# BUBLET/uav-airvision

Measured on AMD Instinct MI355X. Metric: stereo frames/sec (LK+stereo+MSCKF-update) at 752x480, higher is better.
Workload: dtype u8/int32 windows, f32 normal equations

## Files before the change

### uav_airvision_amd/csrc/av_common.h

```cpp
#pragma once
#include <hip/hip_runtime.h>
#include <stdint.h>
#include <stdio.h>
#include <string.h>

#include "../../include/airvision.h"

#define AV_EXPORT extern "C" __attribute__((visibility("default")))

#include "av_resources.h"
#define AV_LAUNCH_CHECK()                                                                         \
    do {                                                                                          \
        hipError_t e_ = hipGetLastError();                                                        \
        if (e_ != hipSuccess) {                                                                   \
            av_set_error("kernel launch failed: %s (%s:%d)", hipGetErrorString(e_), __FILE__, __LINE__); \
            return AV_E_HIP;                                                                      \
        }                                                                                         \
    } while (0)

struct PyrGeom {
    int levels;
    int w[AV_MAX_LEVELS], h[AV_MAX_LEVELS], pitch[AV_MAX_LEVELS];
    int off[AV_MAX_LEVELS];
};
PyrGeom av_make_geom(const av_pyr_layout& l);

struct CamModel {
    double fx, fy, cx, cy, k1, k2, p1, p2;
    int model;
};

#define AV_KP_RASTER_BITS 19
#define AV_KP_RASTER_BITS_WIDE 24
static_assert((1 << AV_KP_RASTER_BITS_WIDE) == AV_MAX_IMAGE_PIXELS, "the wide keypoint word holds every raster of the largest image");
static_assert(((254ull << AV_KP_RASTER_BITS_WIDE) | ((1ull << AV_KP_RASTER_BITS_WIDE) - 1ull)) < 0xFFFFFFFFull, "the largest keypoint word stays below the sentinel");
inline int av_kp_raster_bits(int w, int h) { return (int64_t)w * h <= (1 << AV_KP_RASTER_BITS) ? AV_KP_RASTER_BITS : AV_KP_RASTER_BITS_WIDE; }

#ifdef __HIPCC__
#define AV_HD __host__ __device__
#else
#define AV_HD
#endif
AV_HD inline uint32_t av_ransac_mix(uint32_t x)
{
    x ^= x >> 16; x *= 0x7feb352du; x ^= x >> 15; x *= 0x846ca68bu; x ^= x >> 16;
    return x;
}
AV_HD inline uint32_t av_ransac_hash_inl(uint32_t seed, uint32_t frame, uint32_t camera, uint32_t k, uint32_t draw)
{
    return av_ransac_mix(av_ransac_mix(av_ransac_mix(seed + 0x9e3779b9u) ^ frame) ^ (camera << 16 | k << 1 | draw));
}

#ifdef __HIPCC__
__device__ __forceinline__ void av_mask_box(uint8_t* m, int w, int h, float px, float py, int j, uint8_t val)
{
    int fx = (int)px, fy = (int)py;
    if (fx < 3 || fy < 3) return;
    int yy = fy - 3 + j / 7, xx = fx - 3 + j % 7;
    if (yy < h && xx < w) m[(size_t)yy * w + xx] = val;
}

__device__ __forceinline__ int av_reflect101(int p, int len)
{
    if (p < 0) p = -p;
    if (p >= len) p = 2 * len - 2 - p;
    return p;
}
__device__ __forceinline__ int av_reflect101_any(int p, int len)
{
    if ((unsigned)p < (unsigned)len) return p;
    if (len == 1) return 0;
    do { p = p < 0 ? -p : 2 * len - 2 - p; } while ((unsigned)p >= (unsigned)len);
    return p;
}

__device__ __forceinline__ void av_undistort_fisheye(const CamModel& c, const double* R, double u, double v, double& ox, double& oy)
{
    const double pwx = (u - c.cx) / c.fx, pwy = (v - c.cy) / c.fy;
    const double half_pi = 3.1415926535897932384626433832795 / 2.;
    double theta_d = sqrt(pwx * pwx + pwy * pwy);
    theta_d = fmin(fmax(-half_pi, theta_d), half_pi);
    bool converged = false;
    double theta = theta_d, scale = 0.0;
    if (fabs(theta_d) > 1e-8) {
#pragma unroll 1
        for (int j = 0; j < 10; ++j) {
            const double theta2 = theta * theta, theta4 = theta2 * theta2, theta6 = theta4 * theta2, theta8 = theta6 * theta2;
            const double k0_theta2 = c.k1 * theta2, k1_theta4 = c.k2 * theta4, k2_theta6 = c.p1 * theta6, k3_theta8 = c.p2 * theta8;
            const double theta_fix = (theta * (1 + k0_theta2 + k1_theta4 + k2_theta6 + k3_theta8) - theta_d) /
                                     (1 + 3 * k0_theta2 + 5 * k1_theta4 + 7 * k2_theta6 + 9 * k3_theta8);
            theta = theta - theta_fix;
            if (fabs(theta_fix) < 1e-8) { converged = true; break; }
        }
        scale = tan(theta) / theta_d;
// ... 103 lines not shown
    const int64_t e = av_frame_entry(p, f.g);
    if (e < 0) return false;
    f.src = (f.cam ? p.src1 : p.src0) + (p.src_listed ? e : (int64_t)f.g) * p.src_stride;
    f.dst = (f.cam ? p.dst1 : p.dst0) + e * p.dst_stride;
    return true;
}
#endif

inline bool av_frames_vec16(const FrameSet& src, const FrameSet& dst, int n_groups)
{
    auto al16 = [](const void* p) { return (reinterpret_cast<uintptr_t>(p) & 15) == 0; };
    const bool strides16 = (n_groups == 1 && !src.map && !dst.map) || ((src.stride & 15) == 0 && (dst.stride & 15) == 0);
    return strides16 && al16(src.base[0]) && al16(src.base[1]) && al16(dst.base[0]) && al16(dst.base[1]);
}
inline bool av_spans_overlap(const void* in, int64_t in_stride, int64_t in_bytes, const void* out, int64_t out_stride, int64_t out_bytes, int n)
{
    const uintptr_t i0 = reinterpret_cast<uintptr_t>(in), i1 = i0 + (uint64_t)(n - 1) * in_stride + in_bytes;
    const uintptr_t o0 = reinterpret_cast<uintptr_t>(out), o1 = o0 + (uint64_t)(n - 1) * out_stride + out_bytes;
    return o0 < i1 && i0 < o1;
}

int av_launch_pyramid(const FrameSet& img, int n_groups,
                      const PyrGeom& g, uint8_t* pyr_base, int64_t stream_stride, int64_t slot_stride, int slot0, int slot1,
                      hipStream_t st, bool write_level0 = true, bool* wrote_level0 = nullptr);

struct LKParams {
    int win, max_iter;
    double eps2, min_eig;
};
int av_launch_lk(const ImgView& I, const ImgView& J, int n_set, const PyrGeom& g,
                 const float* prev, float* next, uint8_t* status, const int* count, int cap, int launch_pts,
                 const LKParams& p, hipStream_t st, const int* index = nullptr);

void av_fast_tiles(int w, int h, int* tiles, int* tile_cap);
int av_launch_fast(const ImgView& src, const PyrGeom* g, const uint8_t* mask, int64_t mask_stride,
                   int n_img, int w, int h, int threshold, int raster_bits,
                   uint32_t* kp, int* count, int cap,
                   uint32_t* tile_kp, int* tile_count,
                   int* overflow, int stat_stride, hipStream_t st);

struct RansacStage {
    int S, NT, MAXF, w, h;
    CamModel cam[2];
    const float* prev_p0; const float* prev_p1;
    long long* cur_id; int* cur_life; float* cur_p0; float* cur_p1; int* cur_cell; const int* cur_src; int* cur_count;
    uint8_t* mask;
    const double* Rpc;
    const int* frame_no;
    const int* slot_cur;
    int* counts;
    double thr; int N; uint32_t seed;
};
int av_launch_ransac_stage(const RansacStage& a, hipStream_t st);

int av_clahe_check(int w, int h, double clip_limit, int tiles_x, int tiles_y, const char* who);
int av_launch_clahe(const FrameSet& src, const FrameSet& dst, int n_groups, int w, int h, double clip_limit, int tiles_x, int tiles_y,
                    uint8_t* lut, hipStream_t st);

int av_pixfmt_bytes(int fmt);
int av_pixfmt_packed_depth(int fmt);
bool av_pixfmt_packed_csi2(int fmt);
bool av_pixfmt_is_bayer(int fmt);
const char* av_pixfmt_name(int fmt);
int av_pixfmt_check(int fmt, int shift, const char* who);
int av_pixfmt_check_size(int fmt, int w, int h, const char* who);
int av_launch_to_gray8(const FrameSet& src, const FrameSet& dst, int n_groups, int w, int h, int fmt, int shift, hipStream_t st, const FrameSet* mosaic = nullptr);
int av_launch_unpack_to_gray8(const FrameSet& src, const FrameSet& dst, int n_groups, int w, int h, int fmt, int shift, hipStream_t st);
int av_launch_bayer_to_gray8(const FrameSet& src, const FrameSet& dst, int n_groups, int w, int h, int fmt, int shift, hipStream_t st);
int av_launch_downscale(const FrameSet& src, const FrameSet& dst, int n_groups, int W, int H, int f, hipStream_t st);
int av_launch_photometric(const FrameSet& src, const FrameSet& dst, int n_groups, int w, int h, const uint16_t* resp0, const uint16_t* resp1,
                          const uint16_t* gain0, const uint16_t* gain1, const uint16_t* k0, const uint16_t* k1, hipStream_t st);
struct Range16 {
    int mode, lo, hi, ppm_lo, ppm_hi, min_span;
    uint32_t* hist; uint32_t* rec; int32_t* range_out;
};
int av_range16_check(int mode, int lo, int hi, int ppm_lo, int ppm_hi, int min_span, const char* who);
int av_launch_gray16_range(const FrameSet& src, const FrameSet& dst, int n_groups, int w, int h, const Range16& r, hipStream_t st);
```

### uav_airvision_amd/csrc/fast.hip

```cpp
#include <stdlib.h>

#include "av_common.h"

namespace {

constexpr int TW = 64, TH = 48;
constexpr int PW = TW + 8, PH = TH + 8;
constexpr int PWD = PW / 4;
constexpr int SP = PW, SH = TH + 2;
constexpr int SPD = SP / 4;
constexpr int TCAP = TW * TH / 4;

struct FastArgs {
    const uint8_t* img;
    int64_t img_stride;
    int img_pitch;
    int border;
    const uint8_t* mask;
    int64_t mask_stride;
    int w, h, threshold;
    int rbits;
    uint32_t* kp; int* count; int cap;
    uint32_t* tile_kp; int* tile_count;
    int* overflow; int stat_stride;
    int n_img, tiles_x, tiles_y;
    const int* index;
};

typedef short av_s2 __attribute__((ext_vector_type(2)));
typedef _Float16 av_h2 __attribute__((ext_vector_type(2)));
typedef unsigned short av_us2 __attribute__((ext_vector_type(2)));
__device__ __forceinline__ av_h2 h2_swap(av_h2 x) { return __builtin_shufflevector(x, x, 1, 0); }
__device__ __forceinline__ av_h2 h2_min(av_h2 a, av_h2 b) { return __builtin_elementwise_minimum(a, b); }
__device__ __forceinline__ av_h2 h2_max(av_h2 a, av_h2 b) { return __builtin_elementwise_maximum(a, b); }
__device__ __forceinline__ av_h2 h2_min3(av_h2 a, av_h2 b, av_h2 c) { return __builtin_elementwise_minimum(__builtin_elementwise_minimum(a, b), c); }
__device__ __forceinline__ av_h2 h2_max3(av_h2 a, av_h2 b, av_h2 c) { return __builtin_elementwise_maximum(__builtin_elementwise_maximum(a, b), c); }
__device__ __forceinline__ int fast_score(const uint8_t* c, int t)
{
    constexpr int DX[16] = {0, 1, 2, 3, 3, 3, 2, 1, 0, -1, -2, -3, -3, -3, -2, -1};
// ... 324 lines not shown
```

### uav_airvision_amd/csrc/frontend.hip

```cpp
#include <math.h>

#include <deque>
#include <mutex>
#include <new>
#include <vector>

#include "av_common.h"

namespace {

constexpr int CNT_BEFORE = 0, CNT_TRACKED = 1, CNT_MATCHED = 2, CNT_FAST = 3, CNT_CAND = 4, CNT_NEW = 5, CNT_PUB = 6, CNT_OVF = 7;
constexpr int NCNT = 8;
constexpr unsigned long long LIFE_MAX = 0xFFFFFFull;

struct FeDev {
    int S, w, h, C, grid_row, grid_col, gh, gw, gmin, gmax;
    int MAXF;
    int NT;
    int CC;
    int cell_cap;
    int rbits;
    int NSORT;
    CamModel cam0, cam1;
    double R0to1[9], E[9], I3[9];
    double epi_thr;
    long long* feat_id[2]; int* feat_life[2]; float* feat_p0[2]; float* feat_p1[2]; int* feat_cell[2]; int* n_feat[2];
    long long* next_id; int* first_frame;
    const double* Hmat;
    float* trk_prev; float* trk_next; uint8_t* trk_status; int* trk_count;
    int* sv_src; float* sv_p0; float* sv_init; float* sv_p1; uint8_t* sv_st; float* sv_back; uint8_t* sv_st2; int* sv_count;
    long long* cur_id; int* cur_life; float* cur_p0; float* cur_p1; int* cur_cell; int* cur_count;
    int* cur_src;
    uint32_t* cell_kp; int* cell_count; uint8_t* mask;
    uint32_t* tile_kp; int* tile_count; int n_tiles, tile_cap;
    uint32_t* cand_key; float* cand_p0; float* cand_init; float* cand_p1; uint8_t* cand_st; float* cand_back; uint8_t* cand_st2;
    uint8_t* cand_inl; int* cand_off; int* cand_count;
    int* r1_list; int* r2_list; int* r1_count; int* r2_count;
    long long* out_ids; double* out_uv; int* out_n;
    int* counters;
    const int* slot_cur;
    const uint8_t* smask0; const uint8_t* smask1;
};

__device__ __forceinline__ bool fe_idle(const FeDev& d, int s) { return d.slot_cur != nullptr && d.slot_cur[s] < 0; }

__global__ __launch_bounds__(64) void restart_kernel(FeDev d, const int* list, int n, int* rs_counts)
{
    const int i = blockIdx.x * 64 + threadIdx.x;
    if (i >= n) return;
    const int s = list[i];
    if (s < 0 || s >= d.S) return;
    d.first_frame[s] = 1; d.next_id[s] = 0;
    d.n_feat[0][s] = 0; d.n_feat[1][s] = 0;
    for (int k = 0; k < NCNT; ++k) d.counters[s * NCNT + k] = 0;
    if (rs_counts) for (int k = 0; k < 4; ++k) rs_counts[4 * (size_t)s + k] = 0;
}

__device__ __forceinline__ bool smask_valid(const FeDev& d, const uint8_t* m, float x, float y)
{
    const int xi = min(max((int)x, 0), d.w - 1), yi = min(max((int)y, 0), d.h - 1);
    return m[(size_t)yi * d.w + xi] != 0;
}

__device__ __forceinline__ int cell_of(const FeDev& d, float x, float y)
{
    return (int)(y / (float)d.gh) * d.grid_col + (int)(x / (float)d.gw);
// ... 67 lines not shown
    d.trk_prev[2 * t] = x; d.trk_prev[2 * t + 1] = y;
    d.trk_next[2 * t] = (float)(h0 / h2); d.trk_next[2 * t + 1] = (float)(h1 / h2);
}

__global__ __launch_bounds__(256) void track_gate_kernel(FeDev d)
{
    __shared__ int lds4[4];
    const int s = blockIdx.x;
    if (fe_idle(d, s)) return;
    const int n = d.trk_count[s];
    int base = 0;
    for (int i0 = 0; i0 < n; i0 += NTB) {
        const int i = i0 + threadIdx.x;
        const size_t t = (size_t)s * d.NT + i;
        bool keep = false; float x = 0, y = 0;
        if (i < n) {
            x = d.trk_next[2 * t]; y = d.trk_next[2 * t + 1];
            keep = d.trk_status[t] != 0 && !(x < 0 || x > (float)(d.w - 1) || y < 0 || y > (float)(d.h - 1));
            if (keep && d.smask0) keep = smask_valid(d, d.smask0, x, y);
        }
        int pos = block_ordered_pos(keep, base, lds4);
        if (keep) {
            const size_t o = (size_t)s * d.NT + pos;
            d.sv_src[o] = i;
            d.sv_p0[2 * o] = x; d.sv_p0[2 * o + 1] = y;
            float ix, iy;
            stereo_init(d, x, y, ix, iy);
            d.sv_init[2 * o] = ix; d.sv_init[2 * o + 1] = iy;
            d.sv_p1[2 * o] = ix; d.sv_p1[2 * o + 1] = iy;
            d.sv_back[2 * o] = x; d.sv_back[2 * o + 1] = y;
        }
    }
    if (threadIdx.x == 0) { d.sv_count[s] = base; d.counters[s * NCNT + CNT_TRACKED] = base; }
}

__device__ __forceinline__ void mask_box(const FeDev& d, uint8_t* m, float px, float py, int j, uint8_t val)
{
    av_mask_box(m, d.w, d.h, px, py, j, val);
}

__global__ __launch_bounds__(256) void rebin_kernel(FeDev d, int par)
{
    __shared__ int lds4[4];
    const int s = blockIdx.x;
    if (fe_idle(d, s)) return;
    const int n = d.sv_count[s];
    int base = 0;
    for (int i0 = 0; i0 < n; i0 += NTB) {
        const int i = i0 + threadIdx.x;
        const size_t t = (size_t)s * d.NT + i;
        bool keep = false;
        if (i < n)
            keep = stereo_gate(d, d.sv_p0[2 * t], d.sv_p0[2 * t + 1], d.sv_init[2 * t], d.sv_init[2 * t + 1],
                               d.sv_p1[2 * t], d.sv_p1[2 * t + 1], d.sv_st[t], d.sv_back[2 * t], d.sv_back[2 * t + 1]);
        int pos = block_ordered_pos(keep, base, lds4);
        if (keep) {
            const size_t o = (size_t)s * d.NT + pos;
            const size_t src = (size_t)s * d.MAXF + d.sv_src[t];
            d.cur_id[o] = d.feat_id[par][src];
            d.cur_life[o] = d.feat_life[par][src] + 1;
            float x = d.sv_p0[2 * t], y = d.sv_p0[2 * t + 1];
            d.cur_p0[2 * o] = x; d.cur_p0[2 * o + 1] = y;
            d.cur_p1[2 * o] = d.sv_p1[2 * t]; d.cur_p1[2 * o + 1] = d.sv_p1[2 * t + 1];
            d.cur_cell[o] = cell_of(d, x, y);
            if (d.cur_src) d.cur_src[o] = d.sv_src[t];
        }
    }
    if (threadIdx.x == 0) { d.cur_count[s] = base; d.counters[s * NCNT + CNT_MATCHED] = base; }
    if (d.cur_src) return;
    __syncthreads();
    uint8_t* m = d.mask + (size_t)s * d.w * d.h;
    for (int q = threadIdx.x; q < base * 49; q += NTB) {
        int f = q / 49, j = q - f * 49;
        const size_t o = (size_t)s * d.NT + f;
        mask_box(d, m, d.cur_p0[2 * o], d.cur_p0[2 * o + 1], j, 0);
    }
}

__device__ __forceinline__ unsigned long long wave_max_u64(unsigned long long v)
{
#pragma unroll
    for (int m = 32; m >= 1; m >>= 1) {
        unsigned long long o = __shfl_xor(v, m, 64);
        v = o > v ? o : v;
    }
    return v;
}

__global__ __launch_bounds__(256) void select_kernel(FeDev d)
{
    extern __shared__ int sm[];
    int* cnt = sm;
    int* off = sm + d.C;
    int* ccnt = off + d.C + 1;
    int* tpre = ccnt + d.C;
    const int s = blockIdx.x;
    if (fe_idle(d, s)) return;
    const int ts = d.slot_cur ? d.slot_cur[s] : s;
    const bool first = d.first_frame[s] != 0;
    {
        __shared__ int tmax;
        const int nt = d.n_tiles;
        const uint32_t rmask = (1u << d.rbits) - 1u;
        constexpr int BK = 32, BU = 5;
        if (threadIdx.x == 0) tmax = 0;
        for (int c = threadIdx.x; c < d.C; c += NTB) ccnt[c] = 0;
        __syncthreads();
        int mx = 0;
        for (int t = threadIdx.x; t < nt; t += NTB) { const int n = d.tile_count[(size_t)ts * nt + t]; tpre[t] = n; mx = max(mx, n); }
        if (mx > 0) atomicMax(&tmax, mx);
        __syncthreads();
        const int maxcount = tmax;
        for (int kb = 0; kb < maxcount; kb += BK)
            for (int j0 = threadIdx.x; j0 < nt * BK; j0 += NTB * BU) {
                uint32_t word[BU]; int x[BU], y[BU]; bool ok[BU]; uint8_t mk[BU];
#pragma unroll
                for (int u = 0; u < BU; ++u) {
                    const int j = j0 + NTB * u, t = j / BK, k = kb + (j % BK);
                    ok[u] = j < nt * BK && k < tpre[min(t, nt - 1)];
                    word[u] = ok[u] ? d.tile_kp[((size_t)ts * nt + t) * d.tile_cap + k] : 0u;
                }
#pragma unroll
                for (int u = 0; u < BU; ++u) {
                    const uint32_t raster = rmask - (word[u] & rmask);
                    y[u] = (int)(raster / (uint32_t)d.w); x[u] = (int)(raster % (uint32_t)d.w);
                    mk[u] = ok[u] ? d.mask[(size_t)s * d.w * d.h + (size_t)y[u] * d.w + x[u]] : (uint8_t)0;
                }
#pragma unroll
                for (int u = 0; u < BU; ++u) {
                    if (!ok[u] || mk[u] == 0) continue;
                    const int cell = (y[u] / d.gh) * d.grid_col + x[u] / d.gw;
                    const int idx = atomicAdd(&ccnt[cell], 1);
                    if (idx < d.cell_cap) d.cell_kp[((size_t)s * d.C + cell) * d.cell_cap + idx] = word[u];
                    else atomicOr(&d.counters[s * NCNT + CNT_OVF], 2);
                }
            }
        __threadfence_block();
        __syncthreads();
        if (threadIdx.x == 0) { int tot = 0; for (int c = 0; c < d.C; ++c) tot += ccnt[c]; d.counters[s * NCNT + CNT_FAST] = tot; }
    }
    for (int c = threadIdx.x; c < d.C; c += NTB) {
        int n = min(ccnt[c], d.cell_cap);
        cnt[c] = first ? n : min(n, d.gmax);
    }
    __syncthreads();
    if (threadIdx.x == 0) {
        int acc = 0;
        for (int c = 0; c < d.C; ++c) {
            off[c] = acc;
            int take = cnt[c];
            if (acc + take > d.CC) { take = d.CC - acc; atomicOr(&d.counters[s * NCNT + CNT_OVF], 4); }
            cnt[c] = take;
            acc += take;
        }
        off[d.C] = acc;
        d.cand_count[s] = acc;
        d.counters[s * NCNT + CNT_CAND] = acc;
    }
    __syncthreads();
    for (int c = threadIdx.x; c <= d.C; c += NTB) d.cand_off[s * (d.C + 1) + c] = off[c];
    {
        __shared__ int r1n;
        if (threadIdx.x == 0) r1n = 0;
// ... 189 lines not shown
        const unsigned long long k = keys[j];
        const int c = (int)(k >> 48), ins = (int)(k & 0xFFFFFFull);
        const int rank = j - cell_start[c];
        if (rank >= d.gmax) continue;
        const size_t o = (size_t)s * d.MAXF + out_start[c] + rank;
        if (ins < T) {
            const size_t t = (size_t)s * d.NT + ins;
            d.feat_id[nxt][o] = d.cur_id[t];
            d.feat_life[nxt][o] = d.cur_life[t];
            d.feat_p0[nxt][2 * o] = d.cur_p0[2 * t]; d.feat_p0[nxt][2 * o + 1] = d.cur_p0[2 * t + 1];
            d.feat_p1[nxt][2 * o] = d.cur_p1[2 * t]; d.feat_p1[nxt][2 * o + 1] = d.cur_p1[2 * t + 1];
        } else {
            const size_t q = (size_t)s * d.CC + new_cand[ins - T];
            d.feat_id[nxt][o] = id0 + (ins - T);
            d.feat_life[nxt][o] = 1;
            d.feat_p0[nxt][2 * o] = d.cand_p0[2 * q]; d.feat_p0[nxt][2 * o + 1] = d.cand_p0[2 * q + 1];
            d.feat_p1[nxt][2 * o] = d.cand_p1[2 * q]; d.feat_p1[nxt][2 * o + 1] = d.cand_p1[2 * q + 1];
            flags[0] = 1;
        }
        d.feat_cell[nxt][o] = c;
    }
    __syncthreads();
    const int n_out = out_start[d.C];
    const bool f64 = flags[0] != 0;
    for (int j = threadIdx.x; j < n_out; j += NTB) {
        const size_t o = (size_t)s * d.MAXF + j;
        double u0, v0, u1, v1;
        av_undistort(d.cam0, d.I3, (double)d.feat_p0[nxt][2 * o], (double)d.feat_p0[nxt][2 * o + 1], u0, v0);
        av_undistort(d.cam1, d.I3, (double)d.feat_p1[nxt][2 * o], (double)d.feat_p1[nxt][2 * o + 1], u1, v1);
        if (!f64) { u0 = (double)(float)u0; v0 = (double)(float)v0; }
        d.out_ids[o] = d.feat_id[nxt][o];
        d.out_uv[4 * o] = u0; d.out_uv[4 * o + 1] = v0;
        d.out_uv[4 * o + 2] = (double)(float)u1; d.out_uv[4 * o + 3] = (double)(float)v1;
    }
    uint8_t* m = d.mask + (size_t)s * d.w * d.h;
    for (int q = threadIdx.x; q < T * 49; q += NTB) {
        int f = q / 49, j = q - f * 49;
        const size_t o = (size_t)s * d.NT + f;
        mask_box(d, m, d.cur_p0[2 * o], d.cur_p0[2 * o + 1], j, 1);
    }
    if (threadIdx.x == 0) {
        d.n_feat[nxt][s] = n_out;
        d.out_n[s] = n_out;
        d.next_id[s] = id0 + n_new;
        d.first_frame[s] = 0;
        d.counters[s * NCNT + CNT_NEW] = n_new;
        d.counters[s * NCNT + CNT_PUB] = n_out;
    }
}

struct ImuSample { double t; double w[3]; };

struct StreamHost {
    std::deque<ImuSample> imu;
    std::mutex mu;
    double t_prev = 0.0;
    bool first = true;
    int frame = 0;
};

inline void mat3_mul(const double* A, const double* B, double* o)
{
    for (int i = 0; i < 3; ++i)
        for (int j = 0; j < 3; ++j) o[i * 3 + j] = (A[i * 3 + 0] * B[0 * 3 + j] + A[i * 3 + 1] * B[1 * 3 + j]) + A[i * 3 + 2] * B[2 * 3 + j];
}

inline void rodrigues(const double* r, double* R)
{
    double theta = sqrt((r[0] * r[0] + r[1] * r[1]) + r[2] * r[2]);
    if (theta < 2.220446049250313e-16) { for (int i = 0; i < 9; ++i) R[i] = (i % 4 == 0) ? 1.0 : 0.0; return; }
    double c = cos(theta), s = sin(theta), c1 = 1. - c, it = 1. / theta;
    double x = r[0] * it, y = r[1] * it, z = r[2] * it;
// ... 260 lines not shown
    }
    fe->fed = true;

    auto lk = [&](const ImgView& I, const ImgView& J, const float* prev, float* next, uint8_t* status, const int* count, int cap, int launch_pts, const int* list) -> int {
        Span sp(fe, 1, st);
        return av_launch_lk(I, J, S, fe->geom, prev, next, status, count, cap, launch_pts, fe->lk, st, list);
    };
    auto lk_pair = [&](const ImgView& A, const ImgView& B, const float* p0, float* p1, uint8_t* st1, float* back, uint8_t* st2, const int* count, int cap, int launch_pts, const int* list) -> int {
        const int e = lk(A, B, p0, p1, st1, count, cap, launch_pts, list);
        return e ? e : lk(B, A, p1, back, st2, count, cap, launch_pts, list);
    };
    { Span sp(fe, 3, st);
      hipLaunchKernelGGL(track_prepare_kernel, dim3((d.NT + 255) / 256, S), dim3(256), 0, st, d, par);
      AV_LAUNCH_CHECK(); }
    if ((rc = lk(prev0, cur0, d.trk_prev, d.trk_next, d.trk_status, d.trk_count, d.NT, d.NT, nullptr))) return rc;
    { Span sp(fe, 3, st);
      hipLaunchKernelGGL(track_gate_kernel, dim3(S), dim3(256), 0, st, d);
      AV_LAUNCH_CHECK(); }
    if ((rc = lk_pair(cur0, cur1, d.sv_p0, d.sv_p1, d.sv_st, d.sv_back, d.sv_st2, d.sv_count, d.NT, d.NT, nullptr))) return rc;
    { Span sp(fe, 3, st);
      hipLaunchKernelGGL(rebin_kernel, dim3(S), dim3(256), 0, st, d, par);
      AV_LAUNCH_CHECK(); }
    if (fe->ransac) {
        Span sp(fe, 3, st);
        RansacStage a = fe->rs;
        a.prev_p0 = d.feat_p0[par]; a.prev_p1 = d.feat_p1[par]; a.slot_cur = d.slot_cur;
        if ((rc = av_launch_ransac_stage(a, st))) return rc;
    }
    if (!frames) {
        Span sp(fe, 2, st);
        if ((rc = av_launch_fast(cur0, &fe->geom, d.smask0, 0, S, d.w, d.h, fe->cfg.fast_threshold, d.rbits, nullptr, nullptr, 0, d.tile_kp, d.tile_count, d.counters + CNT_OVF, NCNT, st))) return rc;
    }
    { Span sp(fe, 3, st);
      hipLaunchKernelGGL(select_kernel, dim3(S), dim3(256), sizeof(int) * (3 * d.C + 1 + d.n_tiles + 1), st, d);
      AV_LAUNCH_CHECK(); }
    const int r1_launch = any_first ? d.CC : d.C * (d.gmax < CAND_R1 ? d.gmax : CAND_R1);
    if ((rc = lk_pair(cur0, cur1, d.cand_p0, d.cand_p1, d.cand_st, d.cand_back, d.cand_st2, d.r1_count, d.CC, r1_launch, d.r1_list))) return rc;
    { Span sp(fe, 3, st);
      hipLaunchKernelGGL(cand_round2_kernel, dim3(S), dim3(256), 0, st, d);
      AV_LAUNCH_CHECK(); }
    if (d.gmax > CAND_R1 && (rc = lk_pair(cur0, cur1, d.cand_p0, d.cand_p1, d.cand_st, d.cand_back, d.cand_st2, d.r2_count, d.CC, d.C * (d.gmax - CAND_R1), d.r2_list))) return rc;
    size_t fin_lds = sizeof(unsigned long long) * d.NSORT + sizeof(int) * (2 * d.C * d.gmin + 2 * d.C + 3 * (d.C + 1) + 4);
    { Span sp(fe, 3, st);
      hipLaunchKernelGGL(finalize_kernel, dim3(S), dim3(256), fin_lds, st, d, par);
      AV_LAUNCH_CHECK(); }
    fe->parity = par ^ 1;
    fe->stepped = true; fe->stepped_frames = frames;
    if (frames) { AV_HIP(hipEventRecord(fe->fs.stepped, st)); fe->fs.any_step = true; }
    return AV_OK;
}

}

AV_EXPORT int av_frontend_create(const av_frontend_config* cfg, int n_streams, int device, av_frontend** out)
{
    if (!cfg || !out || n_streams <= 0) { av_set_error("av_frontend_create: bad arguments"); return AV_E_INVALID; }
    if (cfg->width <= 0 || cfg->height <= 0 || (int64_t)cfg->width * cfg->height > AV_MAX_IMAGE_PIXELS) {
        av_set_error("av_frontend_create: the engine takes images of 1 .. AV_MAX_IMAGE_PIXELS = %d pixels (%d x %d)", AV_MAX_IMAGE_PIXELS, cfg->width, cfg->height);
        return AV_E_INVALID;
    }
    if (av_pixfmt_check(cfg->pixel_format, cfg->gray16_shift, "av_frontend_create")) return AV_E_INVALID;
    if (av_pixfmt_check_size(cfg->pixel_format, cfg->width, cfg->height, "av_frontend_create")) return AV_E_INVALID;
    const int in_w = cfg->width, in_h = cfg->height;
    const int ds = cfg->image_downscale == 0 ? 1 : cfg->image_downscale;
    av_frontend_config scaled;
    if ((ds != 1 && ds != 2 && ds != 4) || cfg->reserved1 != 0) {
        av_set_error("av_frontend_create: image_downscale %d is none of 0, 1, 2, 4 (or reserved1 = %d is not 0)", cfg->image_downscale, cfg->reserved1);
// ... 53 lines not shown
    d.gh = (h + cfg->grid_row - 1) / cfg->grid_row;
    d.gw = (w + cfg->grid_col - 1) / cfg->grid_col;
    d.gmin = cfg->grid_min_feature_num; d.gmax = cfg->grid_max_feature_num;
    d.MAXF = C * d.gmax; d.NT = d.MAXF;
    d.CC = cfg->max_corners > C * d.gmax ? cfg->max_corners : C * d.gmax;
    d.cell_cap = (d.gh * d.gw) / 4 + (d.gh + d.gw) / 4 + 64;
    if (d.cell_cap > d.CC) d.cell_cap = d.CC;
    d.rbits = av_kp_raster_bits(w, h);
    int ns = 2; while (ns < C * (d.gmax + d.gmin)) ns <<= 1;
    d.NSORT = ns;
    if (ns > 4096) { av_set_error("av_frontend_create: grid_num*(grid_max+grid_min) = %d exceeds 4096", C * (d.gmax + d.gmin)); delete fe; return AV_E_INVALID; }
    d.cam0 = CamModel{cfg->cam0_intrinsics[0], cfg->cam0_intrinsics[1], cfg->cam0_intrinsics[2], cfg->cam0_intrinsics[3],
                      cfg->cam0_distortion[0], cfg->cam0_distortion[1], cfg->cam0_distortion[2], cfg->cam0_distortion[3], cfg->cam0_distortion_model};
    d.cam1 = CamModel{cfg->cam1_intrinsics[0], cfg->cam1_intrinsics[1], cfg->cam1_intrinsics[2], cfg->cam1_intrinsics[3],
                      cfg->cam1_distortion[0], cfg->cam1_distortion[1], cfg->cam1_distortion[2], cfg->cam1_distortion[3], cfg->cam1_distortion_model};
    for (int i = 0; i < 9; ++i) { d.R0to1[i] = cfg->R0to1[i]; d.E[i] = cfg->E[i]; d.I3[i] = (i % 4 == 0) ? 1.0 : 0.0; }
    d.epi_thr = cfg->stereo_threshold * cfg->norm_unit;

#define A(ptr, n) if ((rc = fe->res.dev(&(ptr), (size_t)(n)))) { av_frontend_destroy(fe); return rc; }
    for (int b = 0; b < 2; ++b) {
        A(d.feat_id[b], S * d.MAXF) A(d.feat_life[b], S * d.MAXF) A(d.feat_p0[b], 2 * S * d.MAXF) A(d.feat_p1[b], 2 * S * d.MAXF)
        A(d.feat_cell[b], S * d.MAXF) A(d.n_feat[b], S)
    }
    A(d.next_id, S)
    if ((rc = fe->res.dev(&d.first_frame, (size_t)S, 1))) { av_frontend_destroy(fe); return rc; }
    A(fe->dH, 9 * S + S + (ransac ? 19 * S : 0))
    d.Hmat = fe->dH;
    A(d.trk_prev, 2 * S * d.NT) A(d.trk_next, 2 * S * d.NT) A(d.trk_status, S * d.NT)
    A(d.sv_src, S * d.NT) A(d.sv_p0, 2 * S * d.NT) A(d.sv_init, 2 * S * d.NT) A(d.sv_p1, 2 * S * d.NT) A(d.sv_st, S * d.NT)
    A(d.sv_back, 2 * S * d.NT) A(d.sv_st2, S * d.NT)
    A(d.cur_id, S * d.NT) A(d.cur_life, S * d.NT) A(d.cur_p0, 2 * S * d.NT) A(d.cur_p1, 2 * S * d.NT) A(d.cur_cell, S * d.NT)
    A(d.cell_kp, (size_t)S * C * d.cell_cap)
    av_fast_tiles(w, h, &d.n_tiles, &d.tile_cap);
    if (sizeof(int) * (size_t)(3 * C + 1 + d.n_tiles + 1) + 64 > 64 * 1024) {
        av_set_error("av_frontend_create: %d x %d has %d detector tiles, more than the selection kernel's LDS holds", w, h, d.n_tiles);
        av_frontend_destroy(fe); return AV_E_INVALID;
    }
    A(d.tile_kp, (size_t)S * d.n_tiles * d.tile_cap) A(d.tile_count, (size_t)S * d.n_tiles)
    if ((rc = fe->res.dev(&d.mask, (size_t)S * w * h, 1))) { av_frontend_destroy(fe); return rc; }
    A(d.cand_key, (size_t)S * d.CC) A(d.cand_p0, 2 * (size_t)S * d.CC) A(d.cand_init, 2 * (size_t)S * d.CC) A(d.cand_p1, 2 * (size_t)S * d.CC)
    A(d.cand_st, (size_t)S * d.CC) A(d.cand_back, 2 * (size_t)S * d.CC) A(d.cand_st2, (size_t)S * d.CC) A(d.cand_inl, (size_t)S * d.CC)
    A(d.cand_off, S * (C + 1))
    A(d.r1_list, (size_t)S * d.CC) A(d.r2_list, (size_t)S * d.CC) A(d.r1_count, S) A(d.r2_count, S)
    A(d.out_ids, S * d.MAXF) A(d.out_uv, 4 * S * d.MAXF) A(d.out_n, S)
    {
        size_t n_int = (size_t)S * 4 + (size_t)S * C + (size_t)S * NCNT;
        int* z = nullptr;
        A(z, n_int)
        fe->zero_region = z; fe->zero_bytes = n_int * sizeof(int);
        d.trk_count = z; d.sv_count = z + S; d.cur_count = z + 2 * S; d.cand_count = z + 3 * S;
        d.cell_count = z + 4 * S; d.counters = z + 4 * S + (size_t)S * C;
    }
    A(fe->pyr, (size_t)S * 3 * fe->lay.bytes)
    if (ransac) {
        A(d.cur_src, S * d.NT) A(fe->rs_counts, 4 * S)
        RansacStage& a = fe->rs;
        memset(&a, 0, sizeof(a));
        a.S = S; a.NT = d.NT; a.MAXF = d.MAXF; a.w = w; a.h = h; a.cam[0] = d.cam0; a.cam[1] = d.cam1;
        a.cur_id = d.cur_id; a.cur_life = d.cur_life; a.cur_p0 = d.cur_p0; a.cur_p1 = d.cur_p1; a.cur_cell = d.cur_cell; a.cur_src = d.cur_src;
        a.cur_count = d.cur_count; a.mask = d.mask; a.counts = fe->rs_counts;
        a.Rpc = fe->dH + (size_t)10 * S; a.frame_no = reinterpret_cast<const int*>(fe->dH + (size_t)28 * S);
        a.thr = cfg->ransac_threshold; a.N = rs_N; a.seed = cfg->ransac_seed;
        fe->ransac = true;
    }
    fe->fmt = cfg->pixel_format; fe->fmt_shift = cfg->gray16_shift;
    fe->ds = ds; fe->in_w = in_w; fe->in_h = in_h; fe->frame_bytes = av_pixfmt_frame_bytes(fe->fmt, in_w, in_h);
    fe->photo_tables = (cfg->flags & AV_FE_PHOTOMETRIC) != 0; fe->expo = (cfg->flags & AV_FE_EXPOSURE) != 0;
    fe->photo = fe->photo_tables || fe->expo;
    fe->own_l0 = clahe || fe->fmt != AV_PIX_GRAY8 || ds > 1 || fe->photo;
    if (fe->own_l0) A(fe->eq, (size_t)3 * S * w * h)
    if (ds > 1 && (fe->fmt != AV_PIX_GRAY8 || fe->photo)) A(fe->gray_full, (size_t)2 * S * in_w * in_h)
    if (fe->photo_tables) A(fe->ph_resp_buf, 2 * 256)
    if (fe->expo) {
        A(fe->ex_d, 2 * S)
        fe->ex_slot_k.assign((size_t)4 * S, 0); fe->ex_last.assign((size_t)2 * S, 0);
    }
    if (av_pixfmt_packed_depth(fe->fmt) && av_pixfmt_is_bayer(fe->fmt)) A(fe->mosaic, (size_t)2 * S * in_w * in_h)
    if (clahe) {
        A(fe->eq_lut, (size_t)2 * S * cfg->clahe_tiles_x * cfg->clahe_tiles_y * 256)
        fe->clahe = true;
    }
#undef A
    rc = fe->hH.create(fe->res, 9 * (size_t)S + S + (ransac ? 19 * (size_t)S : 0));
    if (!rc && fe->expo) rc = fe->ex_h.create(fe->res, 2 * (size_t)S);
    if (!rc && !(rc = fe->rs_h.create(fe->res, (size_t)S))) rc = fe->res.dev(&fe->rs_d, 4 * (size_t)S);
    for (int i = 0; i < 2 && !rc; ++i) {
        av_frontend::ReadSlot& r = fe->rd[i];
        if (!(rc = fe->res.pinned(&r.n, (size_t)S)) && !(rc = fe->res.pinned(&r.ids, (size_t)S * d.MAXF)) && !(rc = fe->res.pinned(&r.uv, 4 * (size_t)S * d.MAXF)) &&
            !(rc = fe->res.pinned(&r.cnt, (size_t)S * NCNT))) rc = fe->res.event(&r.ev, hipEventDisableTiming);
    }
    if (rc) { av_frontend_destroy(fe); return rc; }
    *out = fe;
    return AV_OK;
// ... 629 lines not shown
```

### uav_airvision_amd/csrc/ransac.hip

```cpp
#include <math.h>

#include "av_common.h"

namespace {

constexpr int RS_H = AV_RANSAC_MAX_HYPOTHESES;

__device__ __forceinline__ double rs_wave_sum(double v)
{
#pragma unroll
    for (int m = 32; m >= 1; m >>= 1) v += __shfl_xor(v, m, 64);
    return v;
}
__device__ __forceinline__ unsigned rs_wave_max(unsigned v)
{
#pragma unroll
    for (int m = 32; m >= 1; m >>= 1) { unsigned o = (unsigned)__shfl_xor((int)v, m, 64); v = o > v ? o : v; }
    return v;
}

struct RsResult { int n_set, path; };

template <class Load>
__device__ __forceinline__ RsResult ransac_problem(int n, Load load, const CamModel& cam, const double* R, double thr, int N,
// ... 166 lines not shown
        const float* prev = cam ? a.prev_p1 : a.prev_p0;
        const float* cur = cam ? a.cur_p1 : a.cur_p0;
        const double* Rr = a.Rpc + (size_t)s * 18 + 9 * cam;
        auto load = [&](int i, float& p1x, float& p1y, float& p2x, float& p2y) {
            const size_t src = pb + a.cur_src[cb + i];
            p1x = prev[2 * src]; p1y = prev[2 * src + 1]; p2x = cur[2 * (cb + i)]; p2y = cur[2 * (cb + i) + 1];
        };
        const RsResult r = ransac_problem(n, load, a.cam[cam], Rr, a.thr, a.N, a.seed, frame, (uint32_t)cam, slot, model, mark, (uint8_t)(1 << cam));
        if (cam == 0) { set0 = r.n_set; path = r.path; } else { set1 = r.n_set; path |= r.path << 4; }
    }
    int base = 0;
    for (int i0 = 0; i0 < n; i0 += 64) {
        const int i = i0 + lane;
        const bool keep = i < n && mark[i] == 3;
        long long id = 0; int life = 0, cell = 0; float x0 = 0, y0 = 0, x1 = 0, y1 = 0;
        if (keep) {
            id = a.cur_id[cb + i]; life = a.cur_life[cb + i]; cell = a.cur_cell[cb + i];
            x0 = a.cur_p0[2 * (cb + i)]; y0 = a.cur_p0[2 * (cb + i) + 1]; x1 = a.cur_p1[2 * (cb + i)]; y1 = a.cur_p1[2 * (cb + i) + 1];
        }
        const unsigned long long b = __ballot(keep);
        const int pos = base + __popcll(b & ((1ull << lane) - 1ull));
        __syncthreads();
        if (keep) {
            a.cur_id[cb + pos] = id; a.cur_life[cb + pos] = life; a.cur_cell[cb + pos] = cell;
            a.cur_p0[2 * (cb + pos)] = x0; a.cur_p0[2 * (cb + pos) + 1] = y0; a.cur_p1[2 * (cb + pos)] = x1; a.cur_p1[2 * (cb + pos) + 1] = y1;
        }
        base += __popcll(b);
        __syncthreads();
    }
    if (lane == 0) {
        a.cur_count[s] = base;
        counts[0] = base; counts[1] = set0; counts[2] = set1; counts[3] = path;
    }
    __syncthreads();
    uint8_t* mk = a.mask + (size_t)s * a.w * a.h;
    for (int q = lane; q < base * 49; q += 64) {
        const int f = q / 49, j = q - f * 49;
        av_mask_box(mk, a.w, a.h, a.cur_p0[2 * (cb + f)], a.cur_p0[2 * (cb + f) + 1], j, 0);
    }
}

size_t rs_lds_bytes(int max_pairs) { return ((size_t)max_pairs * 33 + 7) & ~(size_t)7; }

}

int av_launch_ransac_stage(const RansacStage& a, hipStream_t st)
{
    hipLaunchKernelGGL(ransac_stage_kernel, dim3(a.S), dim3(64), rs_lds_bytes(a.NT), st, a);
    AV_LAUNCH_CHECK();
    return AV_OK;
}

AV_EXPORT uint32_t av_ransac_hash(uint32_t seed, uint32_t frame, uint32_t camera, uint32_t k, uint32_t draw)
{
    return av_ransac_hash_inl(seed, frame, camera, k, draw);
}

AV_EXPORT int av_ransac_num_hypotheses(double p)
{
    if (!(p > 0.0 && p < 1.0)) return 0;
    const double v = ceil(log(1.0 - p) / log(1.0 - 0.7 * 0.7));
    if (!(v >= 1.0)) return 1;
    return v > (double)AV_RANSAC_MAX_HYPOTHESES ? AV_RANSAC_MAX_HYPOTHESES : (int)v;
}

AV_EXPORT int av_two_point_ransac(const float* pts1_dev, const float* pts2_dev, const int32_t* off_dev, int n_problems, int max_pairs,
                                  const double* R_dev, const int32_t* camera_dev, const int32_t* frame_dev,
                                  const double* intr, const double* dist, int model, double inlier_error, double success_probability,
                                  uint32_t seed, uint8_t* markers_dev, int32_t* info_dev, void* stream)
{
    if (!off_dev || !R_dev || !intr || !dist || n_problems < 0 || max_pairs < 0 || (max_pairs > 0 && (!pts1_dev || !pts2_dev || !markers_dev))) {
        av_set_error("av_two_point_ransac: bad arguments");
// ... 14 lines not shown
```

Measured before the change: 209,800.

## Replace full-image keep-out mask with per-tile feature box lists in LDS

Removes the per-slot full-resolution byte mask that was cleared and painted with 7x7 boxes around tracked features in several kernels (rebin, ransac, output). Instead, select_kernel buckets tracked feature positions by detector tile in LDS, using a counting pass, a wave prefix scan and a scatter. Each candidate keypoint is then tested against the boxes in its own tile. This drops the global mask writes and the random mask reads, at the cost of extra LDS use that scales with NT and a per-candidate loop over that tile's boxes.

After: 214,400, median of 6. 2.2% higher.

```diff
diff --git a/uav_airvision_amd/csrc/av_common.h b/uav_airvision_amd/csrc/av_common.h
--- a/uav_airvision_amd/csrc/av_common.h
+++ b/uav_airvision_amd/csrc/av_common.h
@@ -52,14 +52,6 @@
 }
 
 #ifdef __HIPCC__
-__device__ __forceinline__ void av_mask_box(uint8_t* m, int w, int h, float px, float py, int j, uint8_t val)
-{
-    int fx = (int)px, fy = (int)py;
-    if (fx < 3 || fy < 3) return;
-    int yy = fy - 3 + j / 7, xx = fx - 3 + j % 7;
-    if (yy < h && xx < w) m[(size_t)yy * w + xx] = val;
-}
-
 __device__ __forceinline__ int av_reflect101(int p, int len)
 {
     if (p < 0) p = -p;
@@ -229,6 +221,7 @@
                  const float* prev, float* next, uint8_t* status, const int* count, int cap, int launch_pts,
                  const LKParams& p, hipStream_t st, const int* index = nullptr);
 
+constexpr int AV_FAST_TW = 64, AV_FAST_TH = 48;
 void av_fast_tiles(int w, int h, int* tiles, int* tile_cap);
 int av_launch_fast(const ImgView& src, const PyrGeom* g, const uint8_t* mask, int64_t mask_stride,
                    int n_img, int w, int h, int threshold, int raster_bits,
@@ -237,11 +230,10 @@
                    int* overflow, int stat_stride, hipStream_t st);
 
 struct RansacStage {
-    int S, NT, MAXF, w, h;
+    int S, NT, MAXF;
     CamModel cam[2];
     const float* prev_p0; const float* prev_p1;
     long long* cur_id; int* cur_life; float* cur_p0; float* cur_p1; int* cur_cell; const int* cur_src; int* cur_count;
-    uint8_t* mask;
     const double* Rpc;
     const int* frame_no;
     const int* slot_cur;
diff --git a/uav_airvision_amd/csrc/fast.hip b/uav_airvision_amd/csrc/fast.hip
--- a/uav_airvision_amd/csrc/fast.hip
+++ b/uav_airvision_amd/csrc/fast.hip
@@ -4,7 +4,7 @@
 
 namespace {
 
-constexpr int TW = 64, TH = 48;
+constexpr int TW = AV_FAST_TW, TH = AV_FAST_TH;
 constexpr int PW = TW + 8, PH = TH + 8;
 constexpr int PWD = PW / 4;
 constexpr int SP = PW, SH = TH + 2;
diff --git a/uav_airvision_amd/csrc/frontend.hip b/uav_airvision_amd/csrc/frontend.hip
--- a/uav_airvision_amd/csrc/frontend.hip
+++ b/uav_airvision_amd/csrc/frontend.hip
@@ -31,7 +31,7 @@
     int* sv_src; float* sv_p0; float* sv_init; float* sv_p1; uint8_t* sv_st; float* sv_back; uint8_t* sv_st2; int* sv_count;
     long long* cur_id; int* cur_life; float* cur_p0; float* cur_p1; int* cur_cell; int* cur_count;
     int* cur_src;
-    uint32_t* cell_kp; int* cell_count; uint8_t* mask;
+    uint32_t* cell_kp; int* cell_count;
     uint32_t* tile_kp; int* tile_count; int n_tiles, tile_cap;
     uint32_t* cand_key; float* cand_p0; float* cand_init; float* cand_p1; uint8_t* cand_st; float* cand_back; uint8_t* cand_st2;
     uint8_t* cand_inl; int* cand_off; int* cand_count;
@@ -165,11 +165,6 @@
         }
     }
     if (threadIdx.x == 0) { d.sv_count[s] = base; d.counters[s * NCNT + CNT_TRACKED] = base; }
-}
-
-__device__ __forceinline__ void mask_box(const FeDev& d, uint8_t* m, float px, float py, int j, uint8_t val)
-{
-    av_mask_box(m, d.w, d.h, px, py, j, val);
 }
 
 __global__ __launch_bounds__(256) void rebin_kernel(FeDev d, int par)
@@ -200,14 +195,6 @@
         }
     }
     if (threadIdx.x == 0) { d.cur_count[s] = base; d.counters[s * NCNT + CNT_MATCHED] = base; }
-    if (d.cur_src) return;
-    __syncthreads();
-    uint8_t* m = d.mask + (size_t)s * d.w * d.h;
-    for (int q = threadIdx.x; q < base * 49; q += NTB) {
-        int f = q / 49, j = q - f * 49;
-        const size_t o = (size_t)s * d.NT + f;
-        mask_box(d, m, d.cur_p0[2 * o], d.cur_p0[2 * o + 1], j, 0);
-    }
 }
 
 __device__ __forceinline__ unsigned long long wave_max_u64(unsigned long long v)
@@ -220,48 +207,97 @@
     return v;
 }
 
+template <class F>
+__device__ __forceinline__ void keepout_tiles(const FeDev& d, int ntx, float px, float py, F f)
+{
+    const int fx = (int)px, fy = (int)py;
+    if (fx < 3 || fy < 3) return;
+    const int tx0 = (fx - 3) / AV_FAST_TW, tx1 = (min(fx, d.w - 4) + 3) / AV_FAST_TW;
+    const int ty0 = (fy - 3) / AV_FAST_TH, ty1 = (min(fy, d.h - 4) + 3) / AV_FAST_TH;
+    for (int ty = ty0; ty <= ty1; ++ty)
+        for (int tx = tx0; tx <= tx1; ++tx)
+            f(ty * ntx + tx, (uint16_t)(((fy - ty * AV_FAST_TH + 3) << 8) | (fx - tx * AV_FAST_TW + 3)));
+}
+static_assert(AV_FAST_TW >= 7 && AV_FAST_TH >= 7 && AV_FAST_TW + 6 <= 256 && AV_FAST_TH + 6 <= 256, "a box touches at most 2 x 2 tiles and its entry is two bytes");
+
+size_t select_lds_bytes(const FeDev& d)
+{
+    return sizeof(int) * (size_t)(3 * d.C + 1 + d.n_tiles + 1) + sizeof(uint16_t) * 4 * (size_t)d.NT;
+}
+static_assert(AV_FAST_TW * AV_FAST_TH / 4 < 65536, "a tile's survivor count fits the low half of its word");
+
 __global__ __launch_bounds__(256) void select_kernel(FeDev d)
 {
     extern __shared__ int sm[];
     int* cnt = sm;
     int* off = sm + d.C;
     int* ccnt = off + d.C + 1;
-    int* tpre = ccnt + d.C;
+    int* tile = ccnt + d.C;
+    uint16_t* box = reinterpret_cast<uint16_t*>(tile + d.n_tiles + 1);
     const int s = blockIdx.x;
     if (fe_idle(d, s)) return;
     const int ts = d.slot_cur ? d.slot_cur[s] : s;
     const bool first = d.first_frame[s] != 0;
     {
         __shared__ int tmax;
-        const int nt = d.n_tiles;
+        const int nt = d.n_tiles, ntx = (d.w + AV_FAST_TW - 1) / AV_FAST_TW;
         const uint32_t rmask = (1u << d.rbits) - 1u;
         constexpr int BK = 32, BU = 5;
         if (threadIdx.x == 0) tmax = 0;
         for (int c = threadIdx.x; c < d.C; c += NTB) ccnt[c] = 0;
+        int mx = 0;
+        for (int t = threadIdx.x; t < nt; t += NTB) { const int n = d.tile_count[(size_t)ts * nt + t]; tile[t] = n; mx = max(mx, n); }
         __syncthreads();
-        int mx = 0;
-        for (int t = threadIdx.x; t < nt; t += NTB) { const int n = d.tile_count[(size_t)ts * nt + t]; tpre[t] = n; mx = max(mx, n); }
         if (mx > 0) atomicMax(&tmax, mx);
+        const int nf = min(d.cur_count[s], d.NT);
+        const float* fp = d.cur_p0 + 2 * (size_t)s * d.NT;
+        if (nf > 0) {
+            for (int i = threadIdx.x; i < nf; i += NTB)
+                keepout_tiles(d, ntx, fp[2 * i], fp[2 * i + 1], [&](int t, uint16_t) { atomicAdd(&tile[t], 1 << 16); });
+            __syncthreads();
+            if (threadIdx.x < 64) {
+                const int lane = threadIdx.x;
+                int carry = 0;
+                for (int t0 = 0; t0 < nt; t0 += 64) {
+                    const int t = t0 + lane, w = t < nt ? tile[t] : 0, v = w >> 16;
+                    int incl = v;
+#pragma unroll
+                    for (int o = 1; o < 64; o <<= 1) { const int up = __shfl_up(incl, o, 64); if (lane >= o) incl += up; }
+                    if (t < nt) tile[t] = (w & 0xFFFF) | ((carry + incl - v) << 16);
+                    carry += __shfl(incl, 63, 64);
+                }
+            }
+            __syncthreads();
+            for (int i = threadIdx.x; i < nf; i += NTB)
+                keepout_tiles(d, ntx, fp[2 * i], fp[2 * i + 1], [&](int t, uint16_t e) { box[atomicAdd(&tile[t], 1 << 16) >> 16] = e; });
+        }
         __syncthreads();
         const int maxcount = tmax;
         for (int kb = 0; kb < maxcount; kb += BK)
             for (int j0 = threadIdx.x; j0 < nt * BK; j0 += NTB * BU) {
-                uint32_t word[BU]; int x[BU], y[BU]; bool ok[BU]; uint8_t mk[BU];
+                uint32_t word[BU]; int x[BU], y[BU]; bool ok[BU];
 #pragma unroll
                 for (int u = 0; u < BU; ++u) {
                     const int j = j0 + NTB * u, t = j / BK, k = kb + (j % BK);
-                    ok[u] = j < nt * BK && k < tpre[min(t, nt - 1)];
+                    ok[u] = j < nt * BK && k < (tile[min(t, nt - 1)] & 0xFFFF);
                     word[u] = ok[u] ? d.tile_kp[((size_t)ts * nt + t) * d.tile_cap + k] : 0u;
                 }
 #pragma unroll
                 for (int u = 0; u < BU; ++u) {
                     const uint32_t raster = rmask - (word[u] & rmask);
                     y[u] = (int)(raster / (uint32_t)d.w); x[u] = (int)(raster % (uint32_t)d.w);
-                    mk[u] = ok[u] ? d.mask[(size_t)s * d.w * d.h + (size_t)y[u] * d.w + x[u]] : (uint8_t)0;
                 }
 #pragma unroll
                 for (int u = 0; u < BU; ++u) {
-                    if (!ok[u] || mk[u] == 0) continue;
+                    if (!ok[u]) continue;
+                    const int t = (j0 + NTB * u) / BK;
+                    const int sx = x[u] % AV_FAST_TW + 6, sy = y[u] % AV_FAST_TH + 6;
+                    bool inside = false;
+                    for (int q = t ? tile[t - 1] >> 16 : 0, qe = tile[t] >> 16; q < qe; ++q) {
+                        const int e = box[q];
+                        inside |= (unsigned)(sx - (e & 0xFF)) <= 6u && (unsigned)(sy - (e >> 8)) <= 6u;
+                    }
+                    if (inside) continue;
                     const int cell = (y[u] / d.gh) * d.grid_col + x[u] / d.gw;
                     const int idx = atomicAdd(&ccnt[cell], 1);
                     if (idx < d.cell_cap) d.cell_kp[((size_t)s * d.C + cell) * d.cell_cap + idx] = word[u];
@@ -517,12 +553,6 @@
         d.out_ids[o] = d.feat_id[nxt][o];
         d.out_uv[4 * o] = u0; d.out_uv[4 * o + 1] = v0;
         d.out_uv[4 * o + 2] = (double)(float)u1; d.out_uv[4 * o + 3] = (double)(float)v1;
-    }
-    uint8_t* m = d.mask + (size_t)s * d.w * d.h;
-    for (int q = threadIdx.x; q < T * 49; q += NTB) {
-        int f = q / 49, j = q - f * 49;
-        const size_t o = (size_t)s * d.NT + f;
-        mask_box(d, m, d.cur_p0[2 * o], d.cur_p0[2 * o + 1], j, 1);
     }
     if (threadIdx.x == 0) {
         d.n_feat[nxt][s] = n_out;
@@ -849,7 +879,7 @@
         if ((rc = av_launch_fast(cur0, &fe->geom, d.smask0, 0, S, d.w, d.h, fe->cfg.fast_threshold, d.rbits, nullptr, nullptr, 0, d.tile_kp, d.tile_count, d.counters + CNT_OVF, NCNT, st))) return rc;
     }
     { Span sp(fe, 3, st);
-      hipLaunchKernelGGL(select_kernel, dim3(S), dim3(256), sizeof(int) * (3 * d.C + 1 + d.n_tiles + 1), st, d);
+      hipLaunchKernelGGL(select_kernel, dim3(S), dim3(256), select_lds_bytes(d), st, d);
       AV_LAUNCH_CHECK(); }
     const int r1_launch = any_first ? d.CC : d.C * (d.gmax < CAND_R1 ? d.gmax : CAND_R1);
     if ((rc = lk_pair(cur0, cur1, d.cand_p0, d.cand_p1, d.cand_st, d.cand_back, d.cand_st2, d.r1_count, d.CC, r1_launch, d.r1_list))) return rc;
@@ -969,12 +999,11 @@
     A(d.cur_id, S * d.NT) A(d.cur_life, S * d.NT) A(d.cur_p0, 2 * S * d.NT) A(d.cur_p1, 2 * S * d.NT) A(d.cur_cell, S * d.NT)
     A(d.cell_kp, (size_t)S * C * d.cell_cap)
     av_fast_tiles(w, h, &d.n_tiles, &d.tile_cap);
-    if (sizeof(int) * (size_t)(3 * C + 1 + d.n_tiles + 1) + 64 > 64 * 1024) {
-        av_set_error("av_frontend_create: %d x %d has %d detector tiles, more than the selection kernel's LDS holds", w, h, d.n_tiles);
+    if (select_lds_bytes(d) + 64 > 64 * 1024) {
+        av_set_error("av_frontend_create: %d x %d has %d detector tiles, with %d features more than the selection kernel's LDS holds", w, h, d.n_tiles, d.NT);
         av_frontend_destroy(fe); return AV_E_INVALID;
     }
     A(d.tile_kp, (size_t)S * d.n_tiles * d.tile_cap) A(d.tile_count, (size_t)S * d.n_tiles)
-    if ((rc = fe->res.dev(&d.mask, (size_t)S * w * h, 1))) { av_frontend_destroy(fe); return rc; }
     A(d.cand_key, (size_t)S * d.CC) A(d.cand_p0, 2 * (size_t)S * d.CC) A(d.cand_init, 2 * (size_t)S * d.CC) A(d.cand_p1, 2 * (size_t)S * d.CC)
     A(d.cand_st, (size_t)S * d.CC) A(d.cand_back, 2 * (size_t)S * d.CC) A(d.cand_st2, (size_t)S * d.CC) A(d.cand_inl, (size_t)S * d.CC)
     A(d.cand_off, S * (C + 1))
@@ -993,9 +1022,9 @@
         A(d.cur_src, S * d.NT) A(fe->rs_counts, 4 * S)
         RansacStage& a = fe->rs;
         memset(&a, 0, sizeof(a));
-        a.S = S; a.NT = d.NT; a.MAXF = d.MAXF; a.w = w; a.h = h; a.cam[0] = d.cam0; a.cam[1] = d.cam1;
+        a.S = S; a.NT = d.NT; a.MAXF = d.MAXF; a.cam[0] = d.cam0; a.cam[1] = d.cam1;
         a.cur_id = d.cur_id; a.cur_life = d.cur_life; a.cur_p0 = d.cur_p0; a.cur_p1 = d.cur_p1; a.cur_cell = d.cur_cell; a.cur_src = d.cur_src;
-        a.cur_count = d.cur_count; a.mask = d.mask; a.counts = fe->rs_counts;
+        a.cur_count = d.cur_count; a.counts = fe->rs_counts;
         a.Rpc = fe->dH + (size_t)10 * S; a.frame_no = reinterpret_cast<const int*>(fe->dH + (size_t)28 * S);
         a.thr = cfg->ransac_threshold; a.N = rs_N; a.seed = cfg->ransac_seed;
         fe->ransac = true;
diff --git a/uav_airvision_amd/csrc/ransac.hip b/uav_airvision_amd/csrc/ransac.hip
--- a/uav_airvision_amd/csrc/ransac.hip
+++ b/uav_airvision_amd/csrc/ransac.hip
@@ -222,12 +222,6 @@
         a.cur_count[s] = base;
         counts[0] = base; counts[1] = set0; counts[2] = set1; counts[3] = path;
     }
-    __syncthreads();
-    uint8_t* mk = a.mask + (size_t)s * a.w * a.h;
-    for (int q = lane; q < base * 49; q += 64) {
-        const int f = q / 49, j = q - f * 49;
-        av_mask_box(mk, a.w, a.h, a.cur_p0[2 * (cb + f)], a.cur_p0[2 * (cb + f) + 1], j, 0);
-    }
 }
 
 size_t rs_lds_bytes(int max_pairs) { return ((size_t)max_pairs * 33 + 7) & ~(size_t)7; }
```
